# MayDomine/Burst-Attention

Hardware: NVIDIA H100
Metric: attention fwd+bwd TFLOPS/s (bs=1, H=32, d=128, bf16; seq in config, default 262144 on N > 1 GPUs, 65536 on one), aggregate over GPUs (higher is better)
Workload: dtype bf16

## Files before the change

### burst-attention_b200/csrc/fwd_sm90.cuh

```cuda
#pragma once
#include <math.h>
#include <stdlib.h>

#include "doc_sm90.cuh"
#include "host_common.h"
#include "sm90_ptx.cuh"

namespace ba {

constexpr int kBlockM = 128;
constexpr int kBlockN = 128;
constexpr int kKStages = 2;
constexpr int kVStages = 2;
constexpr int kBoxBytes = 128 * 64 * 2;
constexpr int kFwdThreads = 384;

struct FwdParams {
  float* o_acc;
  int64_t oacc_sb, oacc_ss, oacc_sh;
  float* lse;
  int64_t lse_sb, lse_sh;
  void* o_out;
  int64_t oout_sb, oout_ss, oout_sh;
  int B, Sq, Sk, H;
  int G;
  float scale_log2;
  const float* bias;
  int64_t bias_sb, bias_sh;
  int causal;
  int causal_off;
  int load_state;
  int store_lowp;
  int lo;
  const float* slopes;
  int64_t slopes_sb;
  int64_t dist0;
  int pstride;
  const int* cu;
  int n_docs;
  int q_pos0, k_pos0;
};

struct __align__(8) FwdBarriers {
  uint64_t q_full;
  uint64_t k_full[kKStages], k_empty[kKStages];
  uint64_t b_full[kKStages];
  uint64_t v_full[kVStages], v_empty[kVStages];
};

template <int kD>
struct FwdLayout {
  static_assert(kD == 64 || kD == 128, "head dim 64 or 128");
  static constexpr uint32_t kTileB = 128 * kD * 2;
  static constexpr int kBoxes = kD / 64;
  static constexpr uint32_t kOffQ = 0;
  static constexpr uint32_t kOffK = kTileB;
  static constexpr uint32_t kOffV = kOffK + kKStages * kTileB;
  static constexpr uint32_t kOffBias = kOffV + kVStages * kTileB;
  static constexpr uint32_t kOffBars = kOffBias + kKStages * kBlockN * 4;
  static constexpr int kSmemBytes = kOffBars + 256 ;
  static_assert(kSmemBytes <= 232448, "forward kernel exceeds 227 KiB of shared memory");
};

__device__ __forceinline__ int fwd_trip_count(int r0, const FwdParams& p) {
  if (r0 >= p.Sq) return 0;
  int r_last = min(r0 + 63, p.Sq - 1);
  int max_limit = p.causal ? min(r_last + p.causal_off, p.Sk - 1) : p.Sk - 1;
  return max_limit < 0 ? 0 : max_limit / kBlockN + 1;
}

__device__ __forceinline__ int fwd_first_tile(int r0, const FwdParams& p) { return max(0, r0 + p.lo) / kBlockN; }

__device__ __forceinline__ void fwd_doc_range(int r0, const FwdParams& p, int* first, int* end) {
  *first = *end = 0;
  if (r0 >= p.Sq) return;
  const int r_last = min(r0 + 63, p.Sq - 1);
  int k_lo, k_hi, unused;
  doc_interval(p.q_pos0 + p.pstride * r0, p.cu, p.n_docs, p.k_pos0, p.pstride, p.Sk, &k_lo, &unused);
  doc_interval(p.q_pos0 + p.pstride * r_last, p.cu, p.n_docs, p.k_pos0, p.pstride, p.Sk, &unused, &k_hi);
  const int f = max(fwd_first_tile(r0, p), k_lo / kBlockN);
  const int e = min(fwd_trip_count(r0, p), (k_hi + kBlockN - 1) / kBlockN);
  if (e > f) *first = f, *end = e;
}

__device__ __forceinline__ int64_t alibi_dref(int a, const FwdParams& p) {
  const int64_t hi = (int64_t)p.pstride * a + p.dist0, lo = hi - (int64_t)p.pstride * (p.Sk - 1);
  return max((int64_t)0, max(lo, -hi));
}

__device__ __forceinline__ int64_t alibi_carried_ref(int64_t dref, float m0, float slope2) {
  if (slope2 > 0.f) {
    const float cap = fmaxf(0.f, -m0) / slope2;
    if (cap < (float)dref) return (int64_t)cap;
  }
  return dref;
}

template <bool kBF16, int kD, bool kBias, bool kBand, bool kAlibi, bool kDoc = false>
__device__ __forceinline__ void fwd_chunk_body(const CUtensorMap& tmQ, const CUtensorMap& tmK, const CUtensorMap& tmV,
                                               const FwdParams& p) {
  static_assert(!(kBias && kAlibi), "ALiBi is not combined with the key bias");
  static_assert(!kDoc || (kBand && !kBias && !kAlibi), "documents run on the band path, without key bias or ALiBi");
  extern __shared__ __align__(1024) uint8_t smem_raw[];
  uint8_t* smem = smem_raw;
  if ((smem_u32(smem) & 1023u) != 0) __trap();
  using L = FwdLayout<kD>;
  constexpr uint32_t kTileBytes = L::kTileB;
  constexpr int kBoxes = L::kBoxes, kOReg = kD / 2;
  uint8_t* sQ = smem + L::kOffQ;
  uint8_t* sK = smem + L::kOffK;
  uint8_t* sV = smem + L::kOffV;
  float* sBias = reinterpret_cast<float*>(smem + L::kOffBias);
  FwdBarriers* bars = reinterpret_cast<FwdBarriers*>(smem + L::kOffBars);

  const int warp = __shfl_sync(0xffffffffu, threadIdx.x >> 5, 0);
  const int lane = threadIdx.x & 31;
  const int h = blockIdx.y, b = blockIdx.z;
  const int row0 = (p.causal ? (int)(gridDim.x - 1 - blockIdx.x) : (int)blockIdx.x) * kBlockM;
  int n_tiles = max(fwd_trip_count(row0, p), fwd_trip_count(row0 + 64, p));
  int t0 = 0;
  if constexpr (kBand) {
    t0 = min(fwd_first_tile(row0, p), n_tiles);
    n_tiles -= t0;
  }
  if constexpr (kDoc) {
    int f0, e0, f1, e1;
    fwd_doc_range(row0, p, &f0, &e0);
    fwd_doc_range(row0 + 64, p, &f1, &e1);
    t0 = e0 > f0 ? (e1 > f1 ? min(f0, f1) : f0) : f1;
    n_tiles = max(0, max(e0, e1) - t0);
  }

  if (threadIdx.x == 0) {
    tma_prefetch_desc(&tmQ);
    tma_prefetch_desc(&tmK);
    tma_prefetch_desc(&tmV);
    mbar_init(&bars->q_full, 1);
    for (int i = 0; i < kKStages; ++i) {
      mbar_init(&bars->k_full[i], 1);
      mbar_init(&bars->k_empty[i], 8);
      mbar_init(&bars->b_full[i], 1);
    }
    for (int i = 0; i < kVStages; ++i) {
      mbar_init(&bars->v_full[i], 1);
      mbar_init(&bars->v_empty[i], 8);
    }
    fence_mbar_init();
  }
  __syncthreads();

  if (warp < 4) {
    reg_alloc_dec<40>();
    if (warp != 0) return;
    const int hk = h / p.G;
    if (lane == 0) {
      mbar_arrive_expect_tx(&bars->q_full, kTileBytes);
      for (int half = 0; half < kBoxes; ++half)
        tma_load_4d(sQ + half * kBoxBytes, &tmQ, &bars->q_full, half * 64, h, row0, b);
    }
    for (int i = 0; i < n_tiles; ++i) {
      const int ks = i % kKStages, kph = (i / kKStages) & 1;
      mbar_wait(&bars->k_empty[ks], kph ^ 1);
      if (lane == 0) {
        mbar_arrive_expect_tx(&bars->k_full[ks], kTileBytes);
        for (int half = 0; half < kBoxes; ++half)
          tma_load_4d(sK + ks * kTileBytes + half * kBoxBytes, &tmK, &bars->k_full[ks], half * 64, hk,
                      (t0 + i) * kBlockN, b);
      }
      if constexpr (kBias) {
#pragma unroll
        for (int j = 0; j < 4; ++j) {
          const int key = (t0 + i) * kBlockN + lane + 32 * j;
          float x = 0.f;
          if (key < p.Sk) x = __ldg(p.bias + (int64_t)b * p.bias_sb + (int64_t)h * p.bias_sh + key) * kLog2e;
          sBias[ks * kBlockN + lane + 32 * j] = x;
        }
        __syncwarp();
        if (lane == 0) mbar_arrive(&bars->b_full[ks]);
      }
      if (lane == 0) {
        const int vs = i % kVStages, vph = (i / kVStages) & 1;
        mbar_wait(&bars->v_empty[vs], vph ^ 1);
        mbar_arrive_expect_tx(&bars->v_full[vs], kTileBytes);
        for (int half = 0; half < kBoxes; ++half)
          tma_load_4d(sV + vs * kTileBytes + half * kBoxBytes, &tmV, &bars->v_full[vs], half * 64, hk,
                      (t0 + i) * kBlockN, b);
      }
      __syncwarp();
    }
    return;
  }

  reg_alloc_inc<232>();
  const int wg = (threadIdx.x >> 7) - 1;
  const int w = warp & 3, g = lane >> 2, t = lane & 3;
  const int r_lo = row0 + wg * 64 + 16 * w + g;
  const int rows[2] = {r_lo, r_lo + 8};
  [[maybe_unused]] int doc_first = 0, doc_end = 0, doc_lo[2] = {0, 0}, doc_hi[2] = {0, 0};
  if constexpr (kDoc) {
    fwd_doc_range(row0 + wg * 64, p, &doc_first, &doc_end);
#pragma unroll
    for (int r = 0; r < 2; ++r)
      if (rows[r] < p.Sq)
        doc_interval(p.q_pos0 + p.pstride * rows[r], p.cu, p.n_docs, p.k_pos0, p.pstride, p.Sk, &doc_lo[r], &doc_hi[r]);
  }
  const int n_mine = kDoc ? doc_end : fwd_trip_count(row0 + wg * 64, p);
  const float scale_log2 = p.scale_log2;
  int limit[2];
#pragma unroll
  for (int r = 0; r < 2; ++r) limit[r] = p.causal ? min(rows[r] + p.causal_off, p.Sk - 1) : p.Sk - 1;
  if constexpr (kDoc) {
#pragma unroll
    for (int r = 0; r < 2; ++r) limit[r] = min(limit[r], doc_hi[r] - 1);
  }
  const int limit_min = min(limit[0], limit[1]);
  int my0 = 0, lo_limit[2] = {0, 0};
  if constexpr (kBand) {
    my0 = fwd_first_tile(row0 + wg * 64, p);
    lo_limit[0] = rows[0] + p.lo;
    lo_limit[1] = rows[1] + p.lo;
  }
  if constexpr (kDoc) {
    my0 = doc_first;
#pragma unroll
    for (int r = 0; r < 2; ++r) lo_limit[r] = max(lo_limit[r], doc_lo[r]);
  }
  const int lo_limit_max = max(lo_limit[0], lo_limit[1]);
  float slope2 = 0.f;
  int64_t dref[2] = {0, 0};
  if constexpr (kAlibi) {
    slope2 = __ldg(p.slopes + (int64_t)b * p.slopes_sb + h) * kLog2e;
    dref[0] = alibi_dref(rows[0], p);
    dref[1] = alibi_dref(rows[1], p);
  }

  float o[kOReg];
  float m[2] = {-INFINITY, -INFINITY}, l[2] = {0.f, 0.f};
#pragma unroll
  for (int i = 0; i < kOReg; ++i) o[i] = 0.f;
  if (p.load_state) {
#pragma unroll
    for (int r = 0; r < 2; ++r) {
      if (rows[r] >= p.Sq) continue;
      const float lse_prev = p.lse[(int64_t)b * p.lse_sb + (int64_t)h * p.lse_sh + rows[r]];
      if (lse_prev != -INFINITY) {
        m[r] = lse_prev * kLog2e;
        if constexpr (kAlibi) {
          dref[r] = alibi_carried_ref(dref[r], m[r], slope2);
          m[r] += slope2 * (float)dref[r];
        }
        l[r] = t == 0 ? 1.f : 0.f;
      }
      const float* src = p.o_acc + (int64_t)b * p.oacc_sb + (int64_t)rows[r] * p.oacc_ss + (int64_t)h * p.oacc_sh;
#pragma unroll
      for (int c = 0; c < kD / 8; ++c) {
        const float2 f = __ldg(reinterpret_cast<const float2*>(src + 8 * c + 2 * t));
        o[4 * c + 2 * r] = f.x;
        o[4 * c + 2 * r + 1] = f.y;
      }
    }
  }

  const uint32_t q_base = smem_u32(sQ) + wg * 64 * 128;
  mbar_wait(&bars->q_full, 0);
  for (int i = 0; i < n_tiles; ++i) {
    const int ks = i % kKStages, kph = (i / kKStages) & 1;
    const int vs = i % kVStages, vph = (i / kVStages) & 1;
    const bool work = kBand ? (t0 + i >= my0 && t0 + i < n_mine) : i < n_mine;
    mbar_wait(&bars->k_full[ks], kph);
    float sc[64];
    if (work) {
      const uint32_t k_base = smem_u32(sK + ks * kTileBytes);
      wgmma_fence();
#pragma unroll
      for (int kk = 0; kk < kD / 16; ++kk) {
        const uint32_t off = (kk >> 2) * kBoxBytes + (kk & 3) * 32;
        wgmma_ss_n128<kBF16, 0, 0>(sc, make_desc(q_base + off, 16, 1024), make_desc(k_base + off, 16, 1024),
                                   kk > 0 ? 1u : 0u);
      }
      wgmma_commit();
      wgmma_wait<0>();
      fence_regs<64>(sc);
      const int key0 = (t0 + i) * kBlockN;
      if constexpr (kBias) {
        mbar_wait(&bars->b_full[ks], kph);
        const float* bias = sBias + ks * kBlockN;
#pragma unroll
        for (int c = 0; c < 16; ++c) {
          const float2 bb = *reinterpret_cast<const float2*>(bias + 8 * c + 2 * t);
#pragma unroll
          for (int r = 0; r < 2; ++r) {
            sc[4 * c + 2 * r] = fmaf(sc[4 * c + 2 * r], scale_log2, bb.x);
            sc[4 * c + 2 * r + 1] = fmaf(sc[4 * c + 2 * r + 1], scale_log2, bb.y);
          }
        }
      } else if constexpr (kAlibi) {
        const int64_t base = (int64_t)p.pstride * (row0 + wg * 64 - key0) + p.dist0;
        const int64_t dmin = base - (int64_t)p.pstride * (kBlockN - 1), dmax = base + (int64_t)p.pstride * 63;
        const float pf = (float)p.pstride;
        if (dmin >= 0 || dmax <= 0) {
          const int sg = dmin >= 0 ? 1 : -1;
          float rowb[2];
#pragma unroll
          for (int r = 0; r < 2; ++r)
            rowb[r] = -slope2 * (float)(sg * ((int64_t)p.pstride * (rows[r] - key0) + p.dist0) - dref[r]);
          const float ks = sg > 0 ? slope2 * pf : -slope2 * pf, kt = ks * (float)(2 * t);
#pragma unroll
          for (int c = 0; c < 16; ++c)
#pragma unroll
            for (int e = 0; e < 4; ++e)
              sc[4 * c + e] = fmaf(sc[4 * c + e], scale_log2, rowb[e >> 1] + fmaf(ks, (float)(8 * c + (e & 1)), kt));
        } else {
          float dr[2], dreff[2];
#pragma unroll
          for (int r = 0; r < 2; ++r) {
            dr[r] = (float)((int64_t)p.pstride * (rows[r] - key0 - 2 * t) + p.dist0);
            dreff[r] = slope2 * (float)dref[r];
          }
#pragma unroll
          for (int c = 0; c < 16; ++c)
#pragma unroll
            for (int e = 0; e < 4; ++e)
              sc[4 * c + e] = fmaf(-slope2, fabsf(fmaf(-pf, (float)(8 * c + (e & 1)), dr[e >> 1])),
                                   fmaf(sc[4 * c + e], scale_log2, dreff[e >> 1]));
        }
      } else {
#pragma unroll
        for (int j = 0; j < 64; ++j) sc[j] *= scale_log2;
      }
      if (key0 + kBlockN - 1 > limit_min) {
#pragma unroll
        for (int c = 0; c < 16; ++c)
#pragma unroll
          for (int e = 0; e < 4; ++e)
            if (key0 + 8 * c + 2 * t + (e & 1) > limit[e >> 1]) sc[4 * c + e] = -INFINITY;
      }
      if constexpr (kBand) {
        if (key0 < lo_limit_max) {
#pragma unroll
          for (int c = 0; c < 16; ++c)
#pragma unroll
            for (int e = 0; e < 4; ++e)
              if (key0 + 8 * c + 2 * t + (e & 1) < lo_limit[e >> 1]) sc[4 * c + e] = -INFINITY;
        }
      }
    }
    __syncwarp();
    if (lane == 0) mbar_arrive(&bars->k_empty[ks]);
    if (work) {
      uint32_t pa[32];
#pragma unroll
      for (int r = 0; r < 2; ++r) {
        float mx = -INFINITY;
#pragma unroll
        for (int c = 0; c < 16; ++c) mx = fmaxf(mx, fmaxf(sc[4 * c + 2 * r], sc[4 * c + 2 * r + 1]));
        mx = fmaxf(mx, __shfl_xor_sync(0xffffffffu, mx, 1));
        mx = fmaxf(mx, __shfl_xor_sync(0xffffffffu, mx, 2));
        const float m_new = fmaxf(m[r], mx);
        const float f = (m[r] == -INFINITY) ? 0.f : ex2(m[r] - m_new);
        const float neg_m = (m_new == -INFINITY) ? 0.f : -m_new;
        m[r] = m_new;
        float sum = 0.f;
#pragma unroll
        for (int c = 0; c < 16; ++c) {
          const float p0 = ex2(sc[4 * c + 2 * r] + neg_m), p1 = ex2(sc[4 * c + 2 * r + 1] + neg_m);
          sc[4 * c + 2 * r] = p0;
          sc[4 * c + 2 * r + 1] = p1;
          sum += p0 + p1;
        }
        l[r] = l[r] * f + sum;
#pragma unroll
        for (int c = 0; c < kD / 8; ++c) {
          o[4 * c + 2 * r] *= f;
          o[4 * c + 2 * r + 1] *= f;
        }
      }
#pragma unroll
      for (int j = 0; j < 32; ++j) pa[j] = pack2<kBF16>(sc[2 * j], sc[2 * j + 1]);
      mbar_wait(&bars->v_full[vs], vph);
      const uint32_t v_base = smem_u32(sV + vs * kTileBytes);
      fence_regs<32>(pa);
      fence_regs<kOReg>(o);
      wgmma_fence();
#pragma unroll
      for (int kk = 0; kk < kBlockN / 16; ++kk) {
        const uint64_t dv = make_desc(v_base + kk * 16 * 128, kBoxBytes, 1024);
        if constexpr (kD == 128) wgmma_rs_n128<kBF16, 1>(o, pa + 4 * kk, dv, 1u);
        else wgmma_rs_n64<kBF16, 1>(o, pa + 4 * kk, dv, 1u);
      }
      wgmma_commit();
      wgmma_wait<0>();
      fence_regs<kOReg>(o);
    } else {
      mbar_wait(&bars->v_full[vs], vph);
    }
    __syncwarp();
    if (lane == 0) mbar_arrive(&bars->v_empty[vs]);
  }

#pragma unroll
  for (int r = 0; r < 2; ++r) {
    float lr = l[r];
    lr += __shfl_xor_sync(0xffffffffu, lr, 1);
    lr += __shfl_xor_sync(0xffffffffu, lr, 2);
    const int row = rows[r];
    if (row >= p.Sq) continue;
    const float inv_l = lr > 0.f ? 1.f / lr : 0.f;
    if constexpr (kAlibi) {
      if (t == 0)
        p.lse[(int64_t)b * p.lse_sb + (int64_t)h * p.lse_sh + row] =
            lr > 0.f ? (m[r] + lg2(lr) - slope2 * (float)dref[r]) * kLn2 : -INFINITY;
    } else {
      if (t == 0) p.lse[(int64_t)b * p.lse_sb + (int64_t)h * p.lse_sh + row] = lr > 0.f ? (m[r] + lg2(lr)) * kLn2 : -INFINITY;
    }
    if (p.store_lowp) {
      uint16_t* dst = reinterpret_cast<uint16_t*>(p.o_out) + (int64_t)b * p.oout_sb + (int64_t)row * p.oout_ss +
                      (int64_t)h * p.oout_sh + 2 * t;
#pragma unroll
      for (int c = 0; c < kD / 8; ++c)
        *reinterpret_cast<uint32_t*>(dst + 8 * c) = pack2<kBF16>(o[4 * c + 2 * r] * inv_l, o[4 * c + 2 * r + 1] * inv_l);
    } else {
      float* dst = p.o_acc + (int64_t)b * p.oacc_sb + (int64_t)row * p.oacc_ss + (int64_t)h * p.oacc_sh + 2 * t;
#pragma unroll
      for (int c = 0; c < kD / 8; ++c)
        *reinterpret_cast<float2*>(dst + 8 * c) = make_float2(o[4 * c + 2 * r] * inv_l, o[4 * c + 2 * r + 1] * inv_l);
    }
  }
}

template <bool kBF16, int kD, bool kBias, bool kBand>
__global__ void __launch_bounds__(kFwdThreads, 1)
fwd_chunk_kernel(const __grid_constant__ CUtensorMap tmQ, const __grid_constant__ CUtensorMap tmK,
                 const __grid_constant__ CUtensorMap tmV, const FwdParams p) {
  fwd_chunk_body<kBF16, kD, kBias, kBand, false>(tmQ, tmK, tmV, p);
}

template <bool kBF16, int kD, bool kBand>
__global__ void __launch_bounds__(kFwdThreads, 1)
fwd_alibi_kernel(const __grid_constant__ CUtensorMap tmQ, const __grid_constant__ CUtensorMap tmK,
                 const __grid_constant__ CUtensorMap tmV, const FwdParams p) {
  fwd_chunk_body<kBF16, kD, false, kBand, true>(tmQ, tmK, tmV, p);
}

template <bool kBF16, int kD>
__global__ void __launch_bounds__(kFwdThreads, 1)
fwd_doc_kernel(const __grid_constant__ CUtensorMap tmQ, const __grid_constant__ CUtensorMap tmK,
               const __grid_constant__ CUtensorMap tmV, const FwdParams p) {
  fwd_chunk_body<kBF16, kD, false, true, false, true>(tmQ, tmK, tmV, p);
}

using FwdKernel = void (*)(CUtensorMap, CUtensorMap, CUtensorMap, FwdParams);

template <bool kBand>
inline FwdKernel fwd_chunk_kernel_of(bool bf16, int D, bool bias) {
  if (bias)
    return D == 64 ? (bf16 ? fwd_chunk_kernel<true, 64, true, kBand> : fwd_chunk_kernel<false, 64, true, kBand>)
                   : (bf16 ? fwd_chunk_kernel<true, 128, true, kBand> : fwd_chunk_kernel<false, 128, true, kBand>);
  return D == 64 ? (bf16 ? fwd_chunk_kernel<true, 64, false, kBand> : fwd_chunk_kernel<false, 64, false, kBand>)
                 : (bf16 ? fwd_chunk_kernel<true, 128, false, kBand> : fwd_chunk_kernel<false, 128, false, kBand>);
}

FwdKernel fwd_band_kernel_of(bool bf16, int D, bool bias);
FwdKernel fwd_alibi_kernel_of(bool bf16, int D, bool band);
FwdKernel fwd_doc_kernel_of(bool bf16, int D);

}
```

### burst-attention_b200/csrc/sm90_ptx.cuh

```cuda
#pragma once
#include <cuda.h>
#include <cuda_bf16.h>
#include <cuda_fp16.h>
#include <cuda_runtime.h>
#include <stdint.h>

namespace ba {

#define BA_DEVICE __device__ __forceinline__

BA_DEVICE uint32_t smem_u32(const void* p) {
  return static_cast<uint32_t>(__cvta_generic_to_shared(p));
}
constexpr float kLog2e = 1.4426950408889634f;
constexpr float kLn2 = 0.6931471805599453f;
BA_DEVICE float ex2(float x) {
  float y;
  asm("ex2.approx.ftz.f32 %0, %1;" : "=f"(y) : "f"(x));
  return y;
}
BA_DEVICE float lg2(float x) {
  float y;
  asm("lg2.approx.ftz.f32 %0, %1;" : "=f"(y) : "f"(x));
  return y;
}
template <int N>
BA_DEVICE void reg_alloc_inc() {
  asm volatile("setmaxnreg.inc.sync.aligned.u32 %0;" ::"n"(N));
}
template <int N>
BA_DEVICE void reg_alloc_dec() {
  asm volatile("setmaxnreg.dec.sync.aligned.u32 %0;" ::"n"(N));
}

BA_DEVICE void mbar_init(uint64_t* bar, uint32_t count) {
  asm volatile("mbarrier.init.shared::cta.b64 [%0], %1;" ::"r"(smem_u32(bar)), "r"(count));
}
BA_DEVICE void fence_mbar_init() { asm volatile("fence.mbarrier_init.release.cluster;" ::: "memory"); }
BA_DEVICE void mbar_arrive(uint64_t* bar) {
  asm volatile("mbarrier.arrive.shared::cta.b64 _, [%0];" ::"r"(smem_u32(bar)) : "memory");
}
BA_DEVICE void mbar_arrive_expect_tx(uint64_t* bar, uint32_t bytes) {
  asm volatile("mbarrier.arrive.expect_tx.shared::cta.b64 _, [%0], %1;" ::"r"(smem_u32(bar)), "r"(bytes)
               : "memory");
}
BA_DEVICE bool mbar_try_wait(uint64_t* bar, uint32_t parity) {
  uint32_t ok;
  asm volatile(
      "{\n\t.reg .pred p;\n\t"
      "mbarrier.try_wait.parity.shared::cta.b64 p, [%1], %2;\n\t"
      "selp.u32 %0, 1, 0, p;\n\t}\n"
      : "=r"(ok)
      : "r"(smem_u32(bar)), "r"(parity)
      : "memory");
  return ok != 0;
}
BA_DEVICE uint64_t global_ns() {
  uint64_t t;
  asm volatile("mov.u64 %0, %%globaltimer;" : "=l"(t));
  return t;
}
BA_DEVICE void mbar_wait(uint64_t* bar, uint32_t parity) {
  if (mbar_try_wait(bar, parity)) return;
#ifdef BA_NO_WATCHDOG
  while (!mbar_try_wait(bar, parity)) {
  }
#else
  const uint64_t t0 = global_ns();
#pragma unroll 1
  for (;;) {
#pragma unroll 1
    for (int i = 0; i < 1024; ++i)
      if (mbar_try_wait(bar, parity)) return;
    if (global_ns() - t0 > 30000000000ull) break;
  }
  __trap();
#endif
}

BA_DEVICE void fence_proxy_async_smem() { asm volatile("fence.proxy.async.shared::cta;" ::: "memory"); }
BA_DEVICE void named_bar_sync(uint32_t id, uint32_t nthreads) {
  asm volatile("bar.sync %0, %1;" ::"r"(id), "r"(nthreads) : "memory");
}

BA_DEVICE void tma_prefetch_desc(const CUtensorMap* m) {
  asm volatile("prefetch.tensormap [%0];" ::"l"(reinterpret_cast<uint64_t>(m)) : "memory");
}
BA_DEVICE void tma_load_4d(void* smem_dst, const CUtensorMap* m, uint64_t* bar, int c0, int c1, int c2,
                           int c3) {
  asm volatile(
      "cp.async.bulk.tensor.4d.shared::cluster.global.mbarrier::complete_tx::bytes"
      " [%0], [%1, {%3, %4, %5, %6}], [%2];"
      :
      : "r"(smem_u32(smem_dst)), "l"(reinterpret_cast<uint64_t>(m)), "r"(smem_u32(bar)), "r"(c0), "r"(c1),
        "r"(c2), "r"(c3)
      : "memory");
}
BA_DEVICE void tma_reduce_add_4d(const CUtensorMap* m, const void* smem_src, int c0, int c1, int c2, int c3) {
  asm volatile(
      "cp.reduce.async.bulk.tensor.4d.global.shared::cta.add.tile.bulk_group [%0, {%2, %3, %4, %5}], [%1];"
      :
      : "l"(reinterpret_cast<uint64_t>(m)), "r"(smem_u32(smem_src)), "r"(c0), "r"(c1), "r"(c2), "r"(c3)
      : "memory");
}
BA_DEVICE void tma_store_commit() { asm volatile("cp.async.bulk.commit_group;" ::: "memory"); }
template <int N>
BA_DEVICE void tma_store_wait_read() {
  asm volatile("cp.async.bulk.wait_group.read %0;" ::"n"(N) : "memory");
}
template <int N>
BA_DEVICE void tma_store_wait() {
  asm volatile("cp.async.bulk.wait_group %0;" ::"n"(N) : "memory");
}

BA_DEVICE uint64_t make_desc(uint32_t smem_addr, uint32_t lbo_bytes, uint32_t sbo_bytes) {
  uint64_t d = 0;
  d |= static_cast<uint64_t>((smem_addr & 0x3FFFF) >> 4);
  d |= static_cast<uint64_t>((lbo_bytes >> 4) & 0x3FFF) << 16;
  d |= static_cast<uint64_t>((sbo_bytes >> 4) & 0x3FFF) << 32;
  d |= static_cast<uint64_t>(1) << 62;
  return d;
}

BA_DEVICE void wgmma_fence() { asm volatile("wgmma.fence.sync.aligned;" ::: "memory"); }
BA_DEVICE void wgmma_commit() { asm volatile("wgmma.commit_group.sync.aligned;" ::: "memory"); }
template <int N>
BA_DEVICE void wgmma_wait() {
  asm volatile("wgmma.wait_group.sync.aligned %0;" ::"n"(N) : "memory");
}
template <int N>
BA_DEVICE void fence_regs(float* r) {
#pragma unroll
  for (int i = 0; i < N; ++i) asm volatile("" : "+f"(r[i])::"memory");
}
template <int N>
BA_DEVICE void fence_regs(uint32_t* r) {
#pragma unroll
  for (int i = 0; i < N; ++i) asm volatile("" : "+r"(r[i])::"memory");
}

#define BA_WGMMA_ACC_64(d) "+f"(d[0]), "+f"(d[1]), "+f"(d[2]), "+f"(d[3]), "+f"(d[4]), "+f"(d[5]), "+f"(d[6]), "+f"(d[7]), "+f"(d[8]), "+f"(d[9]), "+f"(d[10]), "+f"(d[11]), "+f"(d[12]), "+f"(d[13]), "+f"(d[14]), "+f"(d[15]), "+f"(d[16]), "+f"(d[17]), "+f"(d[18]), "+f"(d[19]), "+f"(d[20]), "+f"(d[21]), "+f"(d[22]), "+f"(d[23]), "+f"(d[24]), "+f"(d[25]), "+f"(d[26]), "+f"(d[27]), "+f"(d[28]), "+f"(d[29]), "+f"(d[30]), "+f"(d[31])
#define BA_WGMMA_ACC_128(d) BA_WGMMA_ACC_64(d), "+f"(d[32]), "+f"(d[33]), "+f"(d[34]), "+f"(d[35]), "+f"(d[36]), "+f"(d[37]), "+f"(d[38]), "+f"(d[39]), "+f"(d[40]), "+f"(d[41]), "+f"(d[42]), "+f"(d[43]), "+f"(d[44]), "+f"(d[45]), "+f"(d[46]), "+f"(d[47]), "+f"(d[48]), "+f"(d[49]), "+f"(d[50]), "+f"(d[51]), "+f"(d[52]), "+f"(d[53]), "+f"(d[54]), "+f"(d[55]), "+f"(d[56]), "+f"(d[57]), "+f"(d[58]), "+f"(d[59]), "+f"(d[60]), "+f"(d[61]), "+f"(d[62]), "+f"(d[63])
#define BA_WGMMA_REGS_64 "%0,%1,%2,%3,%4,%5,%6,%7,%8,%9,%10,%11,%12,%13,%14,%15,%16,%17,%18,%19,%20,%21,%22,%23,%24,%25,%26,%27,%28,%29,%30,%31"
#define BA_WGMMA_REGS_128 BA_WGMMA_REGS_64 ",%32,%33,%34,%35,%36,%37,%38,%39,%40,%41,%42,%43,%44,%45,%46,%47,%48,%49,%50,%51,%52,%53,%54,%55,%56,%57,%58,%59,%60,%61,%62,%63"
#define BA_WGMMA_SS(N, TY, A, B, SC, TA, TB)                                                     \
  asm volatile("{\n\t.reg .pred p;\n\t"                                                        \
               "setp.ne.b32 p, %" #SC ", 0;\n\t"                                               \
               "wgmma.mma_async.sync.aligned.m64n" #N "k16.f32." TY "." TY " "                 \
               "{" BA_WGMMA_REGS_##N "}, "                                                      \
               "%" #A ", %" #B ", p, 1, 1, %" #TA ", %" #TB ";\n\t}\n"                         \
               : BA_WGMMA_ACC_##N(d)                                                            \
               : "l"(a_desc), "l"(b_desc), "r"(scale_d), "n"(kTA), "n"(kTB))
#define BA_WGMMA_RS(N, TY, A0, A1, A2, A3, B, SC, TB)                                            \
  asm volatile("{\n\t.reg .pred p;\n\t"                                                        \
               "setp.ne.b32 p, %" #SC ", 0;\n\t"                                               \
               "wgmma.mma_async.sync.aligned.m64n" #N "k16.f32." TY "." TY " "                 \
               "{" BA_WGMMA_REGS_##N "}, "                                                      \
               "{%" #A0 ",%" #A1 ",%" #A2 ",%" #A3 "}, %" #B ", p, 1, 1, %" #TB ";\n\t}\n"     \
               : BA_WGMMA_ACC_##N(d)                                                            \
               : "r"(a[0]), "r"(a[1]), "r"(a[2]), "r"(a[3]), "l"(b_desc), "r"(scale_d), "n"(kTB))

template <bool kBF16, int kTA, int kTB>
BA_DEVICE void wgmma_ss_n64(float* d, uint64_t a_desc, uint64_t b_desc, uint32_t scale_d) {
  if constexpr (kBF16) BA_WGMMA_SS(64, "bf16", 32, 33, 34, 35, 36);
  else BA_WGMMA_SS(64, "f16", 32, 33, 34, 35, 36);
}
template <bool kBF16, int kTB>
BA_DEVICE void wgmma_rs_n64(float* d, const uint32_t* a, uint64_t b_desc, uint32_t scale_d) {
  if constexpr (kBF16) BA_WGMMA_RS(64, "bf16", 32, 33, 34, 35, 36, 37, 38);
  else BA_WGMMA_RS(64, "f16", 32, 33, 34, 35, 36, 37, 38);
}
template <bool kBF16, int kTA, int kTB>
BA_DEVICE void wgmma_ss_n128(float* d, uint64_t a_desc, uint64_t b_desc, uint32_t scale_d) {
  if constexpr (kBF16) BA_WGMMA_SS(128, "bf16", 64, 65, 66, 67, 68);
  else BA_WGMMA_SS(128, "f16", 64, 65, 66, 67, 68);
}
template <bool kBF16, int kTB>
BA_DEVICE void wgmma_rs_n128(float* d, const uint32_t* a, uint64_t b_desc, uint32_t scale_d) {
  if constexpr (kBF16) BA_WGMMA_RS(128, "bf16", 64, 65, 66, 67, 68, 69, 70);
  else BA_WGMMA_RS(128, "f16", 64, 65, 66, 67, 68, 69, 70);
}

template <bool kBF16>
BA_DEVICE uint32_t pack2(float lo, float hi) {
  if constexpr (kBF16) {
    __nv_bfloat162 v = __floats2bfloat162_rn(lo, hi);
    return *reinterpret_cast<uint32_t*>(&v);
  } else {
    __half2 v = __floats2half2_rn(lo, hi);
    return *reinterpret_cast<uint32_t*>(&v);
  }
}

}
```

Before: 503.9.

## Software-pipeline forward QK and PV wgmmas with warpgroup ping-pong scheduling

Restructures the SM90 forward consumer loop so the QK^T wgmma for tile i+1 is issued before the PV wgmma for tile i, letting softmax of the next tile overlap the tensor-core work of the current one (intra-warpgroup pipelining). It also adds named-barrier ping-pong between the two consumer warpgroups so their GEMM issue phases alternate, when both warpgroups have equal trip counts. Tiles outside the work range are now skipped up front with pass_over loops instead of per-iteration predicates. The cost is extra register pressure from holding sc and pa live across stages, plus barrier synchronisation overhead.

```diff
diff --git a/burst-attention_b200/csrc/fwd_sm90.cuh b/burst-attention_b200/csrc/fwd_sm90.cuh
--- a/burst-attention_b200/csrc/fwd_sm90.cuh
+++ b/burst-attention_b200/csrc/fwd_sm90.cuh
@@ -1,6 +1,8 @@
 #pragma once
 #include <math.h>
 #include <stdlib.h>
+
+#include <type_traits>
 
 #include "doc_sm90.cuh"
 #include "host_common.h"
@@ -262,141 +264,214 @@
   }
 
   const uint32_t q_base = smem_u32(sQ) + wg * 64 * 128;
+  auto release_k = [&](int i) {
+    __syncwarp();
+    if (lane == 0) mbar_arrive(&bars->k_empty[i % kKStages]);
+  };
+  auto release_v = [&](int i) {
+    __syncwarp();
+    if (lane == 0) mbar_arrive(&bars->v_empty[i % kVStages]);
+  };
+  auto wait_v = [&](int i) { mbar_wait(&bars->v_full[i % kVStages], (i / kVStages) & 1); };
+  auto issue_s = [&](float* sc, int i) {
+    const uint32_t k_base = smem_u32(sK + (i % kKStages) * kTileBytes);
+    wgmma_fence();
+#pragma unroll
+    for (int kk = 0; kk < kD / 16; ++kk) {
+      const uint32_t off = (kk >> 2) * kBoxBytes + (kk & 3) * 32;
+      wgmma_ss_n128<kBF16, 0, 0>(sc, make_desc(q_base + off, 16, 1024), make_desc(k_base + off, 16, 1024),
+                                 kk > 0 ? 1u : 0u);
+    }
+    wgmma_commit();
+  };
+  auto issue_pv = [&](const uint32_t* pa, int i) {
+    const uint32_t v_base = smem_u32(sV + (i % kVStages) * kTileBytes);
+    wgmma_fence();
+#pragma unroll
+    for (int kk = 0; kk < kBlockN / 16; ++kk) {
+      const uint64_t dv = make_desc(v_base + kk * 16 * 128, kBoxBytes, 1024);
+      if constexpr (kD == 128) wgmma_rs_n128<kBF16, 1>(o, pa + 4 * kk, dv, 1u);
+      else wgmma_rs_n64<kBF16, 1>(o, pa + 4 * kk, dv, 1u);
+    }
+    wgmma_commit();
+  };
+  auto scores = [&](float* sc, int i) {
+    const int ks = i % kKStages;
+    const int key0 = (t0 + i) * kBlockN;
+    if constexpr (kBias) {
+      mbar_wait(&bars->b_full[ks], (i / kKStages) & 1);
+      const float* bias = sBias + ks * kBlockN;
+#pragma unroll
+      for (int c = 0; c < 16; ++c) {
+        const float2 bb = *reinterpret_cast<const float2*>(bias + 8 * c + 2 * t);
+#pragma unroll
+        for (int r = 0; r < 2; ++r) {
+          sc[4 * c + 2 * r] = fmaf(sc[4 * c + 2 * r], scale_log2, bb.x);
+          sc[4 * c + 2 * r + 1] = fmaf(sc[4 * c + 2 * r + 1], scale_log2, bb.y);
+        }
+      }
+    } else if constexpr (kAlibi) {
+      const int64_t base = (int64_t)p.pstride * (row0 + wg * 64 - key0) + p.dist0;
+      const int64_t dmin = base - (int64_t)p.pstride * (kBlockN - 1), dmax = base + (int64_t)p.pstride * 63;
+      const float pf = (float)p.pstride;
+      if (dmin >= 0 || dmax <= 0) {
+        const int sg = dmin >= 0 ? 1 : -1;
+        float rowb[2];
+#pragma unroll
+        for (int r = 0; r < 2; ++r)
+          rowb[r] = -slope2 * (float)(sg * ((int64_t)p.pstride * (rows[r] - key0) + p.dist0) - dref[r]);
+        const float ks = sg > 0 ? slope2 * pf : -slope2 * pf, kt = ks * (float)(2 * t);
+#pragma unroll
+        for (int c = 0; c < 16; ++c)
+#pragma unroll
+          for (int e = 0; e < 4; ++e)
+            sc[4 * c + e] = fmaf(sc[4 * c + e], scale_log2, rowb[e >> 1] + fmaf(ks, (float)(8 * c + (e & 1)), kt));
+      } else {
+        float dr[2], dreff[2];
+#pragma unroll
+        for (int r = 0; r < 2; ++r) {
+          dr[r] = (float)((int64_t)p.pstride * (rows[r] - key0 - 2 * t) + p.dist0);
+          dreff[r] = slope2 * (float)dref[r];
+        }
+#pragma unroll
+        for (int c = 0; c < 16; ++c)
+#pragma unroll
+          for (int e = 0; e < 4; ++e)
+            sc[4 * c + e] = fmaf(-slope2, fabsf(fmaf(-pf, (float)(8 * c + (e & 1)), dr[e >> 1])),
+                                 fmaf(sc[4 * c + e], scale_log2, dreff[e >> 1]));
+      }
+    } else {
+#pragma unroll
+      for (int j = 0; j < 64; ++j) sc[j] *= scale_log2;
+    }
+    if (key0 + kBlockN - 1 > limit_min) {
+#pragma unroll
+      for (int c = 0; c < 16; ++c)
+#pragma unroll
+        for (int e = 0; e < 4; ++e)
+          if (key0 + 8 * c + 2 * t + (e & 1) > limit[e >> 1]) sc[4 * c + e] = -INFINITY;
+    }
+    if constexpr (kBand) {
+      if (key0 < lo_limit_max) {
+#pragma unroll
+        for (int c = 0; c < 16; ++c)
+#pragma unroll
+          for (int e = 0; e < 4; ++e)
+            if (key0 + 8 * c + 2 * t + (e & 1) < lo_limit[e >> 1]) sc[4 * c + e] = -INFINITY;
+      }
+    }
+    release_k(i);
+  };
+  auto softmax = [&](float* sc, float* f) {
+#pragma unroll
+    for (int r = 0; r < 2; ++r) {
+      float mx = -INFINITY;
+#pragma unroll
+      for (int c = 0; c < 16; ++c) mx = fmaxf(mx, fmaxf(sc[4 * c + 2 * r], sc[4 * c + 2 * r + 1]));
+      mx = fmaxf(mx, __shfl_xor_sync(0xffffffffu, mx, 1));
+      mx = fmaxf(mx, __shfl_xor_sync(0xffffffffu, mx, 2));
+      const float m_new = fmaxf(m[r], mx);
+      f[r] = (m[r] == -INFINITY) ? 0.f : ex2(m[r] - m_new);
+      const float neg_m = (m_new == -INFINITY) ? 0.f : -m_new;
+      m[r] = m_new;
+      float sum = 0.f;
+#pragma unroll
+      for (int c = 0; c < 16; ++c) {
+        const float p0 = ex2(sc[4 * c + 2 * r] + neg_m), p1 = ex2(sc[4 * c + 2 * r + 1] + neg_m);
+        sc[4 * c + 2 * r] = p0;
+        sc[4 * c + 2 * r + 1] = p1;
+        sum += p0 + p1;
+      }
+      l[r] = l[r] * f[r] + sum;
+    }
+  };
+  auto rescale_o = [&](const float* f) {
+#pragma unroll
+    for (int r = 0; r < 2; ++r)
+#pragma unroll
+      for (int c = 0; c < kD / 8; ++c) {
+        o[4 * c + 2 * r] *= f[r];
+        o[4 * c + 2 * r + 1] *= f[r];
+      }
+  };
+  auto pack_p = [&](uint32_t* pa, const float* sc) {
+#pragma unroll
+    for (int j = 0; j < 32; ++j) pa[j] = pack2<kBF16>(sc[2 * j], sc[2 * j + 1]);
+  };
+  auto pass_over = [&](int i) {
+    mbar_wait(&bars->k_full[i % kKStages], (i / kKStages) & 1);
+    release_k(i);
+    wait_v(i);
+    release_v(i);
+  };
+
+  const int i_first = min(n_tiles, max(0, my0 - t0));
+  const int i_end = max(i_first, min(n_tiles, n_mine - t0));
   mbar_wait(&bars->q_full, 0);
-  for (int i = 0; i < n_tiles; ++i) {
-    const int ks = i % kKStages, kph = (i / kKStages) & 1;
-    const int vs = i % kVStages, vph = (i / kVStages) & 1;
-    const bool work = kBand ? (t0 + i >= my0 && t0 + i < n_mine) : i < n_mine;
-    mbar_wait(&bars->k_full[ks], kph);
+  for (int i = 0; i < i_first; ++i) pass_over(i);
+  [[maybe_unused]] const auto turn_wait = [&] { named_bar_sync(1 + wg, 256); };
+  [[maybe_unused]] const auto turn_pass = [&] { named_bar_arrive(2 - wg, 256); };
+  auto sweep = [&](auto ping) {
+    constexpr bool kPing = decltype(ping)::value;
     float sc[64];
-    if (work) {
-      const uint32_t k_base = smem_u32(sK + ks * kTileBytes);
-      wgmma_fence();
-#pragma unroll
-      for (int kk = 0; kk < kD / 16; ++kk) {
-        const uint32_t off = (kk >> 2) * kBoxBytes + (kk & 3) * 32;
-        wgmma_ss_n128<kBF16, 0, 0>(sc, make_desc(q_base + off, 16, 1024), make_desc(k_base + off, 16, 1024),
-                                   kk > 0 ? 1u : 0u);
-      }
-      wgmma_commit();
-      wgmma_wait<0>();
-      fence_regs<64>(sc);
-      const int key0 = (t0 + i) * kBlockN;
-      if constexpr (kBias) {
-        mbar_wait(&bars->b_full[ks], kph);
-        const float* bias = sBias + ks * kBlockN;
-#pragma unroll
-        for (int c = 0; c < 16; ++c) {
-          const float2 bb = *reinterpret_cast<const float2*>(bias + 8 * c + 2 * t);
-#pragma unroll
-          for (int r = 0; r < 2; ++r) {
-            sc[4 * c + 2 * r] = fmaf(sc[4 * c + 2 * r], scale_log2, bb.x);
-            sc[4 * c + 2 * r + 1] = fmaf(sc[4 * c + 2 * r + 1], scale_log2, bb.y);
-          }
-        }
-      } else if constexpr (kAlibi) {
-        const int64_t base = (int64_t)p.pstride * (row0 + wg * 64 - key0) + p.dist0;
-        const int64_t dmin = base - (int64_t)p.pstride * (kBlockN - 1), dmax = base + (int64_t)p.pstride * 63;
-        const float pf = (float)p.pstride;
-        if (dmin >= 0 || dmax <= 0) {
-          const int sg = dmin >= 0 ? 1 : -1;
-          float rowb[2];
-#pragma unroll
-          for (int r = 0; r < 2; ++r)
-            rowb[r] = -slope2 * (float)(sg * ((int64_t)p.pstride * (rows[r] - key0) + p.dist0) - dref[r]);
-          const float ks = sg > 0 ? slope2 * pf : -slope2 * pf, kt = ks * (float)(2 * t);
-#pragma unroll
-          for (int c = 0; c < 16; ++c)
-#pragma unroll
-            for (int e = 0; e < 4; ++e)
-              sc[4 * c + e] = fmaf(sc[4 * c + e], scale_log2, rowb[e >> 1] + fmaf(ks, (float)(8 * c + (e & 1)), kt));
-        } else {
-          float dr[2], dreff[2];
-#pragma unroll
-          for (int r = 0; r < 2; ++r) {
-            dr[r] = (float)((int64_t)p.pstride * (rows[r] - key0 - 2 * t) + p.dist0);
-            dreff[r] = slope2 * (float)dref[r];
-          }
-#pragma unroll
-          for (int c = 0; c < 16; ++c)
-#pragma unroll
-            for (int e = 0; e < 4; ++e)
-              sc[4 * c + e] = fmaf(-slope2, fabsf(fmaf(-pf, (float)(8 * c + (e & 1)), dr[e >> 1])),
-                                   fmaf(sc[4 * c + e], scale_log2, dreff[e >> 1]));
-        }
-      } else {
-#pragma unroll
-        for (int j = 0; j < 64; ++j) sc[j] *= scale_log2;
-      }
-      if (key0 + kBlockN - 1 > limit_min) {
-#pragma unroll
-        for (int c = 0; c < 16; ++c)
-#pragma unroll
-          for (int e = 0; e < 4; ++e)
-            if (key0 + 8 * c + 2 * t + (e & 1) > limit[e >> 1]) sc[4 * c + e] = -INFINITY;
-      }
-      if constexpr (kBand) {
-        if (key0 < lo_limit_max) {
-#pragma unroll
-          for (int c = 0; c < 16; ++c)
-#pragma unroll
-            for (int e = 0; e < 4; ++e)
-              if (key0 + 8 * c + 2 * t + (e & 1) < lo_limit[e >> 1]) sc[4 * c + e] = -INFINITY;
-        }
-      }
-    }
-    __syncwarp();
-    if (lane == 0) mbar_arrive(&bars->k_empty[ks]);
-    if (work) {
-      uint32_t pa[32];
-#pragma unroll
-      for (int r = 0; r < 2; ++r) {
-        float mx = -INFINITY;
-#pragma unroll
-        for (int c = 0; c < 16; ++c) mx = fmaxf(mx, fmaxf(sc[4 * c + 2 * r], sc[4 * c + 2 * r + 1]));
-        mx = fmaxf(mx, __shfl_xor_sync(0xffffffffu, mx, 1));
-        mx = fmaxf(mx, __shfl_xor_sync(0xffffffffu, mx, 2));
-        const float m_new = fmaxf(m[r], mx);
-        const float f = (m[r] == -INFINITY) ? 0.f : ex2(m[r] - m_new);
-        const float neg_m = (m_new == -INFINITY) ? 0.f : -m_new;
-        m[r] = m_new;
-        float sum = 0.f;
-#pragma unroll
-        for (int c = 0; c < 16; ++c) {
-          const float p0 = ex2(sc[4 * c + 2 * r] + neg_m), p1 = ex2(sc[4 * c + 2 * r + 1] + neg_m);
-          sc[4 * c + 2 * r] = p0;
-          sc[4 * c + 2 * r + 1] = p1;
-          sum += p0 + p1;
-        }
-        l[r] = l[r] * f + sum;
-#pragma unroll
-        for (int c = 0; c < kD / 8; ++c) {
-          o[4 * c + 2 * r] *= f;
-          o[4 * c + 2 * r + 1] *= f;
-        }
-      }
-#pragma unroll
-      for (int j = 0; j < 32; ++j) pa[j] = pack2<kBF16>(sc[2 * j], sc[2 * j + 1]);
-      mbar_wait(&bars->v_full[vs], vph);
-      const uint32_t v_base = smem_u32(sV + vs * kTileBytes);
+    uint32_t pa[32];
+    float f[2];
+    if constexpr (kPing) {
+      if (wg == 1) turn_pass();
+    }
+    mbar_wait(&bars->k_full[i_first % kKStages], (i_first / kKStages) & 1);
+    if constexpr (kPing) turn_wait();
+    issue_s(sc, i_first);
+    if constexpr (kPing) turn_pass();
+    wgmma_wait<0>();
+    fence_regs<64>(sc);
+    scores(sc, i_first);
+    softmax(sc, f);
+    rescale_o(f);
+    pack_p(pa, sc);
+    wait_v(i_first);
+    auto step = [&](auto next, int i) {
+      constexpr bool kNext = decltype(next)::value;
+      if constexpr (kNext) mbar_wait(&bars->k_full[(i + 1) % kKStages], ((i + 1) / kKStages) & 1);
+      if constexpr (kPing) turn_wait();
+      if constexpr (kNext) issue_s(sc, i + 1);
       fence_regs<32>(pa);
       fence_regs<kOReg>(o);
-      wgmma_fence();
-#pragma unroll
-      for (int kk = 0; kk < kBlockN / 16; ++kk) {
-        const uint64_t dv = make_desc(v_base + kk * 16 * 128, kBoxBytes, 1024);
-        if constexpr (kD == 128) wgmma_rs_n128<kBF16, 1>(o, pa + 4 * kk, dv, 1u);
-        else wgmma_rs_n64<kBF16, 1>(o, pa + 4 * kk, dv, 1u);
-      }
-      wgmma_commit();
+      issue_pv(pa, i);
+      if constexpr (kPing) turn_pass();
+      if constexpr (kNext) {
+        wgmma_wait<1>();
+        fence_regs<64>(sc);
+        scores(sc, i + 1);
+        softmax(sc, f);
+        fence_regs<64>(sc);
+        wait_v(i + 1);
+      }
       wgmma_wait<0>();
       fence_regs<kOReg>(o);
+      release_v(i);
+      if constexpr (kNext) {
+        fence_regs<64>(sc);
+        rescale_o(f);
+        pack_p(pa, sc);
+      }
+    };
+#pragma unroll 1
+    for (int i = i_first; i < i_end - 1; ++i) step(std::true_type(), i);
+    step(std::false_type(), i_end - 1);
+    if constexpr (kPing) {
+      if (wg == 0) turn_wait();
+    }
+  };
+  if (i_end > i_first) {
+    if constexpr (!kBand) {
+      if (fwd_trip_count(row0, p) == fwd_trip_count(row0 + 64, p)) sweep(std::true_type());
+      else sweep(std::false_type());
     } else {
-      mbar_wait(&bars->v_full[vs], vph);
-    }
-    __syncwarp();
-    if (lane == 0) mbar_arrive(&bars->v_empty[vs]);
-  }
+      sweep(std::false_type());
+    }
+  }
+  for (int i = i_end; i < n_tiles; ++i) pass_over(i);
 
 #pragma unroll
   for (int r = 0; r < 2; ++r) {
diff --git a/burst-attention_b200/csrc/sm90_ptx.cuh b/burst-attention_b200/csrc/sm90_ptx.cuh
--- a/burst-attention_b200/csrc/sm90_ptx.cuh
+++ b/burst-attention_b200/csrc/sm90_ptx.cuh
@@ -81,6 +81,9 @@
 BA_DEVICE void fence_proxy_async_smem() { asm volatile("fence.proxy.async.shared::cta;" ::: "memory"); }
 BA_DEVICE void named_bar_sync(uint32_t id, uint32_t nthreads) {
   asm volatile("bar.sync %0, %1;" ::"r"(id), "r"(nthreads) : "memory");
+}
+BA_DEVICE void named_bar_arrive(uint32_t id, uint32_t nthreads) {
+  asm volatile("bar.arrive %0, %1;" ::"r"(id), "r"(nthreads) : "memory");
 }
 
 BA_DEVICE void tma_prefetch_desc(const CUtensorMap* m) {
```

After: 507.6, median of 6. About the same (+0.7%).

## Software-pipeline forward loop: overlap next QK^T wgmma with previous PV wgmma

Applied to the files above, without the earlier changes.

Restructures the forward consumer loop so that tile i's S=QK^T wgmma is issued together with tile i-1's PV wgmma. The softmax of tile i then runs while PV(i-1) is still in flight, following the FA3-style intra-warpgroup overlap. Idle tiles before and after the active range are split into a separate barrier-only loop, and a volatile shared store is added to pin instruction ordering before the wait. This costs more registers live at once (sc, pa and o together) and deferred rescaling of o, which risks spills or scheduling changes.

```diff
diff --git a/burst-attention_b200/csrc/fwd_sm90.cuh b/burst-attention_b200/csrc/fwd_sm90.cuh
--- a/burst-attention_b200/csrc/fwd_sm90.cuh
+++ b/burst-attention_b200/csrc/fwd_sm90.cuh
@@ -1,6 +1,8 @@
 #pragma once
 #include <math.h>
 #include <stdlib.h>
+
+#include <type_traits>
 
 #include "doc_sm90.cuh"
 #include "host_common.h"
@@ -58,7 +60,8 @@
   static constexpr uint32_t kOffV = kOffK + kKStages * kTileB;
   static constexpr uint32_t kOffBias = kOffV + kVStages * kTileB;
   static constexpr uint32_t kOffBars = kOffBias + kKStages * kBlockN * 4;
-  static constexpr int kSmemBytes = kOffBars + 256 ;
+  static constexpr uint32_t kOffSink = kOffBars + 256 ;
+  static constexpr int kSmemBytes = kOffSink + 256 * 8;
   static_assert(kSmemBytes <= 232448, "forward kernel exceeds 227 KiB of shared memory");
 };
 
@@ -261,26 +264,61 @@
     }
   }
 
+  const int ia = min(max(my0 - t0, 0), n_tiles), ie = min(max(n_mine - t0, ia), n_tiles);
+
   const uint32_t q_base = smem_u32(sQ) + wg * 64 * 128;
-  mbar_wait(&bars->q_full, 0);
-  for (int i = 0; i < n_tiles; ++i) {
+  const uint32_t sink = smem_u32(smem + L::kOffSink) + (threadIdx.x - 128) * 8;
+  float sc[64];
+  uint32_t pa[32];
+  float f[2];
+
+  auto idle = [&](int i) {
     const int ks = i % kKStages, kph = (i / kKStages) & 1;
     const int vs = i % kVStages, vph = (i / kVStages) & 1;
-    const bool work = kBand ? (t0 + i >= my0 && t0 + i < n_mine) : i < n_mine;
     mbar_wait(&bars->k_full[ks], kph);
-    float sc[64];
-    if (work) {
-      const uint32_t k_base = smem_u32(sK + ks * kTileBytes);
-      wgmma_fence();
-#pragma unroll
-      for (int kk = 0; kk < kD / 16; ++kk) {
-        const uint32_t off = (kk >> 2) * kBoxBytes + (kk & 3) * 32;
-        wgmma_ss_n128<kBF16, 0, 0>(sc, make_desc(q_base + off, 16, 1024), make_desc(k_base + off, 16, 1024),
-                                   kk > 0 ? 1u : 0u);
-      }
-      wgmma_commit();
-      wgmma_wait<0>();
-      fence_regs<64>(sc);
+    __syncwarp();
+    if (lane == 0) mbar_arrive(&bars->k_empty[ks]);
+    mbar_wait(&bars->v_full[vs], vph);
+    __syncwarp();
+    if (lane == 0) mbar_arrive(&bars->v_empty[vs]);
+  };
+  auto issue_s = [&](int i) {
+    const int ks = i % kKStages, kph = (i / kKStages) & 1;
+    mbar_wait(&bars->k_full[ks], kph);
+    const uint32_t k_base = smem_u32(sK + ks * kTileBytes);
+    wgmma_fence();
+#pragma unroll
+    for (int kk = 0; kk < kD / 16; ++kk) {
+      const uint32_t off = (kk >> 2) * kBoxBytes + (kk & 3) * 32;
+      wgmma_ss_n128<kBF16, 0, 0>(sc, make_desc(q_base + off, 16, 1024), make_desc(k_base + off, 16, 1024),
+                                 kk > 0 ? 1u : 0u);
+    }
+    wgmma_commit();
+  };
+  auto issue_pv = [&](int j) {
+    const int vs = j % kVStages, vph = (j / kVStages) & 1;
+    mbar_wait(&bars->v_full[vs], vph);
+    const uint32_t v_base = smem_u32(sV + vs * kTileBytes);
+    wgmma_fence();
+#pragma unroll
+    for (int kk = 0; kk < kBlockN / 16; ++kk) {
+      const uint64_t dv = make_desc(v_base + kk * 16 * 128, kBoxBytes, 1024);
+      if constexpr (kD == 128) wgmma_rs_n128<kBF16, 1>(o, pa + 4 * kk, dv, 1u);
+      else wgmma_rs_n64<kBF16, 1>(o, pa + 4 * kk, dv, 1u);
+    }
+    wgmma_commit();
+  };
+
+  auto step = [&](auto first, int i) {
+    constexpr bool kFirst = decltype(first)::value;
+    const int ks = i % kKStages;
+    [[maybe_unused]] const int kph = (i / kKStages) & 1;
+    fence_regs<64>(sc);
+    issue_s(i);
+    if constexpr (!kFirst) issue_pv(i - 1);
+    wgmma_wait<kFirst ? 0 : 1>();
+    fence_regs<64>(sc);
+    {
       const int key0 = (t0 + i) * kBlockN;
       if constexpr (kBias) {
         mbar_wait(&bars->b_full[ks], kph);
@@ -347,56 +385,58 @@
     }
     __syncwarp();
     if (lane == 0) mbar_arrive(&bars->k_empty[ks]);
-    if (work) {
-      uint32_t pa[32];
-#pragma unroll
-      for (int r = 0; r < 2; ++r) {
-        float mx = -INFINITY;
-#pragma unroll
-        for (int c = 0; c < 16; ++c) mx = fmaxf(mx, fmaxf(sc[4 * c + 2 * r], sc[4 * c + 2 * r + 1]));
-        mx = fmaxf(mx, __shfl_xor_sync(0xffffffffu, mx, 1));
-        mx = fmaxf(mx, __shfl_xor_sync(0xffffffffu, mx, 2));
-        const float m_new = fmaxf(m[r], mx);
-        const float f = (m[r] == -INFINITY) ? 0.f : ex2(m[r] - m_new);
-        const float neg_m = (m_new == -INFINITY) ? 0.f : -m_new;
-        m[r] = m_new;
-        float sum = 0.f;
-#pragma unroll
-        for (int c = 0; c < 16; ++c) {
-          const float p0 = ex2(sc[4 * c + 2 * r] + neg_m), p1 = ex2(sc[4 * c + 2 * r + 1] + neg_m);
-          sc[4 * c + 2 * r] = p0;
-          sc[4 * c + 2 * r + 1] = p1;
-          sum += p0 + p1;
-        }
-        l[r] = l[r] * f + sum;
-#pragma unroll
-        for (int c = 0; c < kD / 8; ++c) {
-          o[4 * c + 2 * r] *= f;
-          o[4 * c + 2 * r + 1] *= f;
-        }
-      }
-#pragma unroll
-      for (int j = 0; j < 32; ++j) pa[j] = pack2<kBF16>(sc[2 * j], sc[2 * j + 1]);
-      mbar_wait(&bars->v_full[vs], vph);
-      const uint32_t v_base = smem_u32(sV + vs * kTileBytes);
-      fence_regs<32>(pa);
-      fence_regs<kOReg>(o);
-      wgmma_fence();
-#pragma unroll
-      for (int kk = 0; kk < kBlockN / 16; ++kk) {
-        const uint64_t dv = make_desc(v_base + kk * 16 * 128, kBoxBytes, 1024);
-        if constexpr (kD == 128) wgmma_rs_n128<kBF16, 1>(o, pa + 4 * kk, dv, 1u);
-        else wgmma_rs_n64<kBF16, 1>(o, pa + 4 * kk, dv, 1u);
-      }
-      wgmma_commit();
+#pragma unroll
+    for (int r = 0; r < 2; ++r) {
+      float mx = -INFINITY;
+#pragma unroll
+      for (int c = 0; c < 16; ++c) mx = fmaxf(mx, fmaxf(sc[4 * c + 2 * r], sc[4 * c + 2 * r + 1]));
+      mx = fmaxf(mx, __shfl_xor_sync(0xffffffffu, mx, 1));
+      mx = fmaxf(mx, __shfl_xor_sync(0xffffffffu, mx, 2));
+      const float m_new = fmaxf(m[r], mx);
+      f[r] = (m[r] == -INFINITY) ? 0.f : ex2(m[r] - m_new);
+      const float neg_m = (m_new == -INFINITY) ? 0.f : -m_new;
+      m[r] = m_new;
+      float sum = 0.f;
+#pragma unroll
+      for (int c = 0; c < 16; ++c) {
+        const float p0 = ex2(sc[4 * c + 2 * r] + neg_m), p1 = ex2(sc[4 * c + 2 * r + 1] + neg_m);
+        sc[4 * c + 2 * r] = p0;
+        sc[4 * c + 2 * r + 1] = p1;
+        sum += p0 + p1;
+      }
+      l[r] = l[r] * f[r] + sum;
+    }
+    if constexpr (!kFirst) {
+      fence_regs<64>(sc);
+      pin_before_wait(sink, l[0], l[1]);
       wgmma_wait<0>();
       fence_regs<kOReg>(o);
-    } else {
-      mbar_wait(&bars->v_full[vs], vph);
-    }
+      fence_regs<64>(sc);
+      __syncwarp();
+      if (lane == 0) mbar_arrive(&bars->v_empty[(i - 1) % kVStages]);
+    }
+#pragma unroll
+    for (int c = 0; c < kD / 8; ++c)
+#pragma unroll
+      for (int e = 0; e < 4; ++e) o[4 * c + e] *= f[e >> 1];
+#pragma unroll
+    for (int j = 0; j < 32; ++j) pa[j] = pack2<kBF16>(sc[2 * j], sc[2 * j + 1]);
+    fence_regs<32>(pa);
+    fence_regs<kOReg>(o);
+  };
+
+  mbar_wait(&bars->q_full, 0);
+  for (int i = 0; i < ia; ++i) idle(i);
+  if (ie > ia) {
+    step(std::true_type(), ia);
+    for (int i = ia + 1; i < ie; ++i) step(std::false_type(), i);
+    issue_pv(ie - 1);
+    wgmma_wait<0>();
+    fence_regs<kOReg>(o);
     __syncwarp();
-    if (lane == 0) mbar_arrive(&bars->v_empty[vs]);
-  }
+    if (lane == 0) mbar_arrive(&bars->v_empty[(ie - 1) % kVStages]);
+  }
+  for (int i = ie; i < n_tiles; ++i) idle(i);
 
 #pragma unroll
   for (int r = 0; r < 2; ++r) {
diff --git a/burst-attention_b200/csrc/sm90_ptx.cuh b/burst-attention_b200/csrc/sm90_ptx.cuh
--- a/burst-attention_b200/csrc/sm90_ptx.cuh
+++ b/burst-attention_b200/csrc/sm90_ptx.cuh
@@ -138,6 +138,9 @@
 #pragma unroll
   for (int i = 0; i < N; ++i) asm volatile("" : "+r"(r[i])::"memory");
 }
+BA_DEVICE void pin_before_wait(uint32_t slot, float a, float b) {
+  asm volatile("st.volatile.shared.v2.f32 [%0], {%1, %2};" ::"r"(slot), "f"(a), "f"(b) : "memory");
+}
 
 #define BA_WGMMA_ACC_64(d) "+f"(d[0]), "+f"(d[1]), "+f"(d[2]), "+f"(d[3]), "+f"(d[4]), "+f"(d[5]), "+f"(d[6]), "+f"(d[7]), "+f"(d[8]), "+f"(d[9]), "+f"(d[10]), "+f"(d[11]), "+f"(d[12]), "+f"(d[13]), "+f"(d[14]), "+f"(d[15]), "+f"(d[16]), "+f"(d[17]), "+f"(d[18]), "+f"(d[19]), "+f"(d[20]), "+f"(d[21]), "+f"(d[22]), "+f"(d[23]), "+f"(d[24]), "+f"(d[25]), "+f"(d[26]), "+f"(d[27]), "+f"(d[28]), "+f"(d[29]), "+f"(d[30]), "+f"(d[31])
 #define BA_WGMMA_ACC_128(d) BA_WGMMA_ACC_64(d), "+f"(d[32]), "+f"(d[33]), "+f"(d[34]), "+f"(d[35]), "+f"(d[36]), "+f"(d[37]), "+f"(d[38]), "+f"(d[39]), "+f"(d[40]), "+f"(d[41]), "+f"(d[42]), "+f"(d[43]), "+f"(d[44]), "+f"(d[45]), "+f"(d[46]), "+f"(d[47]), "+f"(d[48]), "+f"(d[49]), "+f"(d[50]), "+f"(d[51]), "+f"(d[52]), "+f"(d[53]), "+f"(d[54]), "+f"(d[55]), "+f"(d[56]), "+f"(d[57]), "+f"(d[58]), "+f"(d[59]), "+f"(d[60]), "+f"(d[61]), "+f"(d[62]), "+f"(d[63])
```

New measurement: 507.3 before, 499.9 after, median of 6. 0.985x the previous value.
